# 0xPolygon/go-ibft

Hardware: AMD Instinct MI355X
Metric: committed_seal_verifies_per_sec (higher is better)
Workload: dtype u32

## Files before the change

### go-ibft_amd/build.py

```python
from __future__ import annotations

import os
import subprocess

HERE = os.path.dirname(os.path.abspath(__file__))
CSRC = os.path.join(HERE, "csrc")
LIB = os.path.join(CSRC, "libibftgpu.so")
SOURCES = ["ibftgpu.hip", "kernels.hip.h", "recover_dev.h", "verify_dev.h", "wave_fe_dev.h", "wire_dev.h", "cert_wave_dev.h", "modinv_dev.h",
           "sign_dev.h", "secp256k1_dev.h", "keccak_dev.h", os.path.join("..", "..", "include", "ibftgpu.h")]
CODEGEN_FLAGS = ["-mllvm", "-amdgpu-sched-strategy=max-ilp"]
EXTRA_FLAGS = ([] if os.environ.get("IBFT_NO_CODEGEN_FLAGS") == "1" else CODEGEN_FLAGS) + os.environ.get("IBFT_HIPCC_FLAGS", "").split()
HOST_HARNESS = os.path.join(CSRC, "libdev_arith_host.so")
WAVE_HARNESS = os.path.join(CSRC, "libdev_wave_host.so")
CERT_WAVE_HARNESS = os.path.join(CSRC, "libdev_cert_wave_host.so")


def _digest(deps: list[str], extra: str = "") -> str:
    import hashlib
    h = hashlib.sha256(extra.encode())
    for d in deps:
        with open(os.path.join(CSRC, d), "rb") as f:
            h.update(d.encode() + b"\0" + f.read() + b"\0")
    return h.hexdigest()


def _file_sha256(path: str) -> str:
    import hashlib
    h = hashlib.sha256()
    with open(path, "rb") as f:
        for blk in iter(lambda: f.read(1 << 20), b""):
            h.update(blk)
    return h.hexdigest()


def _read_stamp(target: str) -> list[str]:
    try:
        with open(target + ".stamp") as f:
            return f.read().split("\n")
    except OSError:
        return []


# ... 50 lines not shown


def build_lib(force: bool = False, verbose: bool = False) -> str:
    cmd = ["hipcc", "--offload-arch=gfx950", "-O3", "-std=c++17", *EXTRA_FLAGS, "-shared", "-fPIC",
           "-o", LIB, os.path.join(CSRC, "ibftgpu.hip"), "-ldl"]
    stamp_extra = " ".join(cmd[:-3]) + (" +phase_align" if PHASE_ALIGN else "")
    deps = SOURCES + ([os.path.join("..", "phase_align.py")] if PHASE_ALIGN else [])
    retry = PHASE_ALIGN and (build_info(LIB)["flavour"] or "").startswith("phase_align_failed")
    if force or retry or _stale(LIB, deps, stamp_extra):
        done = False
        flavour = "one_step"
        if PHASE_ALIGN:
            try:
                if verbose:
                    print(" ".join(cmd), "  (+ phase_align.py between device assembly and code object)", flush=True)
                _build_lib_phase_aligned(verbose)
                done = True
                flavour = "phase_align"
            except Exception as e:
                print(f"build: phase-aligned build failed ({e}); building with hipcc in one step", flush=True)
                flavour = "phase_align_failed: " + " ".join(str(e).split())[:300]
        if not done:
            if verbose:
                print(" ".join(cmd), flush=True)
            subprocess.check_call(cmd, cwd=CSRC)
        _mark(LIB, deps, stamp_extra, flavour)
    return LIB


DEVTEST = os.path.join(CSRC, "libibft_devtest.so")


def build_devtest(force: bool = False) -> str:
    deps = ["devtest.hip", "recover_dev.h", "modinv_dev.h", "secp256k1_dev.h", "keccak_dev.h", "wave_fe_dev.h", "verify_dev.h"]
    if force or _stale(DEVTEST, deps):
        subprocess.check_call(["hipcc", "--offload-arch=gfx950", "-O3", "-std=c++17", "-shared", "-fPIC", "-w",
                               "-o", DEVTEST, os.path.join(CSRC, "devtest.hip")], cwd=CSRC)
        _mark(DEVTEST, deps)
    return DEVTEST


def build_host_harness(force: bool = False) -> str:
    deps = ["host_arith_harness.hip", "sign_dev.h", "recover_dev.h", "modinv_dev.h", "secp256k1_dev.h", "keccak_dev.h", "wire_dev.h", "verify_dev.h"]
    if force or _stale(HOST_HARNESS, deps):
        subprocess.check_call(["hipcc", "--cuda-host-only", "-O2", "-std=c++17", "-shared", "-fPIC",
                               "-o", HOST_HARNESS, os.path.join(CSRC, "host_arith_harness.hip")], cwd=CSRC)
        _mark(HOST_HARNESS, deps)
    return HOST_HARNESS


def build_wave_harness(force: bool = False) -> str:
    deps = ["host_wave_harness.hip", "wave_fe_dev.h", "wave_emul.h", "recover_dev.h", "verify_dev.h",
            "modinv_dev.h", "secp256k1_dev.h", "keccak_dev.h"]
    if force or _stale(WAVE_HARNESS, deps):
        subprocess.check_call(["hipcc", "--cuda-host-only", "-O2", "-std=c++17", "-shared", "-fPIC",
                               "-o", WAVE_HARNESS, os.path.join(CSRC, "host_wave_harness.hip")], cwd=CSRC)
        _mark(WAVE_HARNESS, deps)
    return WAVE_HARNESS


def build_cert_wave_harness(force: bool = False) -> str:
    deps = ["host_cert_wave_harness.hip", "cert_wave_dev.h", "wave_emul.h", "wire_dev.h", "keccak_dev.h"]
    if force or _stale(CERT_WAVE_HARNESS, deps):
        subprocess.check_call(["hipcc", "--cuda-host-only", "-O2", "-std=c++17", "-shared", "-fPIC",
                               "-o", CERT_WAVE_HARNESS, os.path.join(CSRC, "host_cert_wave_harness.hip")], cwd=CSRC)
        _mark(CERT_WAVE_HARNESS, deps)
    return CERT_WAVE_HARNESS


PROPOSAL_DIGEST_HARNESS = os.path.join(CSRC, "libdev_proposal_digest_host.so")


def build_proposal_digest_harness(force: bool = False) -> str:
    deps = ["host_proposal_digest_harness.hip", "cert_wave_dev.h", "wave_emul.h", "wire_dev.h", "keccak_dev.h"]
    if force or _stale(PROPOSAL_DIGEST_HARNESS, deps):
        subprocess.check_call(["hipcc", "--cuda-host-only", "-O2", "-std=c++17", "-shared", "-fPIC",
                               "-o", PROPOSAL_DIGEST_HARNESS, os.path.join(CSRC, "host_proposal_digest_harness.hip")], cwd=CSRC)
        _mark(PROPOSAL_DIGEST_HARNESS, deps)
    return PROPOSAL_DIGEST_HARNESS


BLOCK_SETS_HARNESS = os.path.join(CSRC, "libdev_block_sets_host.so")


def build_block_sets_harness(force: bool = False) -> str:
    deps = ["host_block_sets_harness.hip", "recover_dev.h", "modinv_dev.h", "secp256k1_dev.h", "keccak_dev.h"]
    if force or _stale(BLOCK_SETS_HARNESS, deps):
        subprocess.check_call(["hipcc", "--cuda-host-only", "-O2", "-std=c++17", "-shared", "-fPIC",
                               "-o", BLOCK_SETS_HARNESS, os.path.join(CSRC, "host_block_sets_harness.hip")], cwd=CSRC)
        _mark(BLOCK_SETS_HARNESS, deps)
    return BLOCK_SETS_HARNESS


BLOCK_HEAD_HARNESS = os.path.join(CSRC, "libdev_block_head_host.so")


def build_block_head_harness(force: bool = False) -> str:
    deps = ["host_block_head_harness.hip", "recover_dev.h", "modinv_dev.h", "secp256k1_dev.h", "keccak_dev.h"]
    if force or _stale(BLOCK_HEAD_HARNESS, deps):
        subprocess.check_call(["hipcc", "--cuda-host-only", "-O2", "-std=c++17", "-shared", "-fPIC",
                               "-o", BLOCK_HEAD_HARNESS, os.path.join(CSRC, "host_block_head_harness.hip")], cwd=CSRC)
        _mark(BLOCK_HEAD_HARNESS, deps)
# ... 6 lines not shown
```

### go-ibft_amd/csrc/devtest.hip

```cpp
#include <hip/hip_runtime.h>
#include <stdint.h>

#include "modinv_dev.h"
#include "recover_dev.h"
#include "secp256k1_dev.h"

using namespace secp;

__global__ void devtest_kernel(int op, int n, const uint8_t *a, const uint8_t *b, uint8_t *out) {
  int i = blockIdx.x * blockDim.x + threadIdx.x;
  if (i >= n) return;
  u256 x = from_be32(a + 32 * i), y = from_be32(b + 32 * i);
  u256 r = zero256();
  switch (op) {
    case 0: r = fe_to_u256(fe_mul(fe_from_u256(x), fe_from_u256(y))); break;
    case 1: r = fe_to_u256(fe_sqr(fe_from_u256(x))); break;
    case 2: r = fe_to_u256(fe_inv(fe_from_u256(x))); break;
    case 3: r = fe_to_u256(fe_inv_safegcd(fe_from_u256(x))); break;
    case 4: r = sc_canon(sc_mul(sc_from_u256(x), sc_from_u256(y))); break;
    case 5: r = sc_canon(sc_inv(sc_from_u256(x))); break;
    case 6: r = sc_canon(sc_inv_safegcd(sc_from_u256(x))); break;
    case 7: r = fe_to_u256(fe_sqrt_candidate(fe_from_u256(x))); break;
    case 8: {
      glv_split s = sc_split_lambda(x);
// ... 131 lines not shown
}
__device__ __forceinline__ wv::wjac devtest_load_pt(const uint32_t *src, const wv::wk &k) {
  const uint32_t *r = src + 31 * k.row;
  wv::wjac p;
  p.x = k.li < 10 ? r[k.li] : 0u;
  p.y = k.li < 10 ? r[10 + k.li] : 0u;
  p.z = k.li < 10 ? r[20 + k.li] : 0u;
  p.inf = r[30] != 0;
  return p;
}
__global__ void __launch_bounds__(64) devtest_wave_pt_kernel(int op, const uint32_t *pp, const uint32_t *qq, uint32_t *out) {
  const wv::wk k = wv::wk_init();
  wv::wjac p = devtest_load_pt(pp + 124 * blockIdx.x, k), q = devtest_load_pt(qq + 124 * blockIdx.x, k), r;
  switch (op) {
    case 0: r = wv::wjac_dbl(p, k); break;
    case 1: r = wv::wjac_add(p, q, k); break;
    case 2: r = wv::wjac_add_aff(p, wv::waff{q.x, q.y}, k); break;
    default: r = wv::wjac_add(p, wv::wjac_lane_xor(p, 16), k); break;
  }
  uint32_t *o = out + 124 * blockIdx.x + 31 * k.row;
  if (k.li < 10) {
    o[k.li] = r.x;
    o[10 + k.li] = r.y;
    o[20 + k.li] = r.z;
  }
  if (k.li == 0) o[30] = r.inf ? 1u : 0u;
}
template <int STOP>
__global__ void __launch_bounds__(64) devtest_wave_recover_kernel(const uint32_t *gtab, const uint8_t *dig, const uint8_t *sig65,
                                                                uint32_t flags, uint8_t *out) {
  const int i = blockIdx.x;
  uint32_t addr[5] = {0, 0, 0, 0, 0};
  aff Q;
  bool ok = wv::recover_pubkey_wave<STOP>(gtab, from_be32(dig + 32 * i), from_be32(sig65 + 65 * i), from_be32(sig65 + 65 * i + 32),
                                    sig65[65 * i + 64], flags, addr, Q);
  uint8_t *o = out + (size_t)24 * (64 * i + threadIdx.x);
  for (int k = 0; k < 5; k++) reinterpret_cast<uint32_t *>(o)[k] = addr[k];
  o[20] = ok ? 1 : 0;
}

template <typename T>
static T *dev_copy(const T *h, size_t n) {
  T *d = nullptr;
  if (hipMalloc(&d, n * sizeof(T)) != hipSuccess) return nullptr;
  (void)hipMemcpy(d, h, n * sizeof(T), hipMemcpyHostToDevice);
  return d;
}
extern "C" int devtest_wave_fe(int op, int jobs, const uint32_t *a, const uint32_t *b, uint32_t *out) {
  uint32_t *da = dev_copy(a, (size_t)40 * jobs), *db = dev_copy(b, (size_t)40 * jobs), *dout;
  if (!da || !db || hipMalloc(&dout, (size_t)256 * jobs) != hipSuccess) return -1;
  devtest_wave_fe_kernel<<<jobs, 64>>>(op, da, db, dout);
  int rc = hipDeviceSynchronize() == hipSuccess ? 0 : -2;
  (void)hipMemcpy(out, dout, (size_t)256 * jobs, hipMemcpyDeviceToHost);
  (void)hipFree(da); (void)hipFree(db); (void)hipFree(dout);
  return rc;
}
extern "C" int devtest_wave_pt(int op, int jobs, const uint32_t *p, const uint32_t *q, uint32_t *out) {
  uint32_t *dp = dev_copy(p, (size_t)124 * jobs), *dq = dev_copy(q, (size_t)124 * jobs), *dout;
  if (!dp || !dq || hipMalloc(&dout, (size_t)496 * jobs) != hipSuccess) return -1;
  (void)hipMemset(dout, 0, (size_t)496 * jobs);
  devtest_wave_pt_kernel<<<jobs, 64>>>(op, dp, dq, dout);
  int rc = hipDeviceSynchronize() == hipSuccess ? 0 : -2;
  (void)hipMemcpy(out, dout, (size_t)496 * jobs, hipMemcpyDeviceToHost);
  (void)hipFree(dp); (void)hipFree(dq); (void)hipFree(dout);
  return rc;
}
extern "C" int devtest_wave_recover(int n, const uint8_t *dig, const uint8_t *sig65, uint32_t flags, uint8_t *out) {
  uint32_t *dg;
// ... 110 lines not shown
  if (!dd || !ds || hipMalloc(&dout, (size_t)24 * n) != hipSuccess) return -1;
  devtest_gtab_kernel<<<(ibftk::GTAB_WINDOWS * ibftk::GTAB_ENTRIES + 63) / 64, 64>>>(dg);
  hipEvent_t e0, e1;
  (void)hipEventCreate(&e0); (void)hipEventCreate(&e1);
  const int waves = (n + 3) / 4, blocks = (waves + 3) / 4;
  for (int reps = 1; reps <= max_reps; reps++)
    for (int t = 0; t < 3; t++) {
      (void)hipEventRecord(e0, 0);
      devtest_rows_repeat_kernel<<<blocks, 256>>>(dg, dd, ds, (uint32_t)n, reps, dout);
      (void)hipEventRecord(e1, 0);
      (void)hipEventSynchronize(e1);
      (void)hipEventElapsedTime(&ms[reps - 1], e0, e1);
    }
  int rc = hipDeviceSynchronize() == hipSuccess ? 0 : -2;
  (void)hipFree(dd); (void)hipFree(ds); (void)hipFree(dout); (void)hipFree(dg);
  return rc;
}

struct stamp_sync {
  uint64_t *st;
  uint32_t *cnt;
  __device__ void operator()() const {
    const uint64_t a = __builtin_amdgcn_s_memrealtime();
    __syncthreads();
    const uint64_t b = __builtin_amdgcn_s_memrealtime();
    if (__lane_id() == 0) {
      const uint32_t i = *cnt;
      st[1 + 2 * i] = a;
      st[2 + 2 * i] = b;
      *cnt = i + 1;
    }
  }
};
__global__ void __launch_bounds__(512) devtest_rows_pair_kernel(const uint32_t *gtab, const uint8_t *dig, const uint8_t *sig65,
                                                              uint32_t n, uint8_t *out, uint64_t *stamps) {
  __shared__ uint32_t row_tab[4][wv::ROW_TAB_SLOTS * 64];
  __shared__ wv::rows_pair_shared sh[4];
  __shared__ uint32_t cnt[8];
  const uint32_t w = threadIdx.x >> 6, lane = threadIdx.x & 63u, slot = w & 3u;
  uint64_t *st = stamps + (size_t)(blockIdx.x * 8 + w) * 8;
  if (lane == 0) {
    cnt[w] = 0;
    st[0] = __builtin_amdgcn_s_memrealtime();
  }
  const stamp_sync sync{st, &cnt[w]};
  const uint32_t row_raw = (blockIdx.x * 4 + slot) * 4u + (lane >> 4);
  const uint32_t i = row_raw < n ? row_raw : n - 1;
  const u256 r = from_be32(sig65 + 65 * i), s = from_be32(sig65 + 65 * i + 32);
  if (w >= 4) {
    wv::recover_helper_row(gtab, from_be32(dig + 32 * i), r, s, &sh[slot], sync);
    if (lane == 0) st[5] = __builtin_amdgcn_s_memrealtime();
    return;
  }
  uint32_t addr[5] = {0, 0, 0, 0, 0};
  aff Q;
  const bool ok = wv::recover_pubkey_row<99, true>(gtab, zero256(), r, s, sig65[65 * i + 64], 0, addr, Q, row_tab[slot], &sh[slot], sync);
  if (lane == 0) st[5] = __builtin_amdgcn_s_memrealtime();
  if ((lane & 15u) == 0 && row_raw < n) {
    uint8_t *o = out + (size_t)24 * i;
    for (int k = 0; k < 5; k++) reinterpret_cast<uint32_t *>(o)[k] = addr[k];
    o[20] = ok ? 1 : 0;
  }
}
extern "C" int devtest_rows_pair_stamps(int n, const uint8_t *dig, const uint8_t *sig65, uint8_t *out24, uint64_t *stamps8,
                                        float *ms) {
  if (n <= 0 || n % 16 != 0) return -3;
  uint32_t *dg;
  size_t gbytes = (size_t)ibftk::GTAB_WINDOWS * ibftk::GTAB_ENTRIES * ibftk::GTAB_ENTRY_DWORDS * 4;
  if (hipMalloc(&dg, gbytes) != hipSuccess) return -1;
  const int blocks = n / 16;
  const size_t st_words = (size_t)blocks * 8 * 8;
  uint8_t *dd = dev_copy(dig, (size_t)32 * n), *ds = dev_copy(sig65, (size_t)65 * n), *dout;
  uint64_t *dst;
  if (!dd || !ds || hipMalloc(&dout, (size_t)24 * n) != hipSuccess || hipMalloc(&dst, st_words * 8) != hipSuccess) return -1;
  devtest_gtab_kernel<<<(ibftk::GTAB_WINDOWS * ibftk::GTAB_ENTRIES + 63) / 64, 64>>>(dg);
  hipEvent_t e0, e1;
  (void)hipEventCreate(&e0); (void)hipEventCreate(&e1);
  for (int rep = 0; rep < 3; rep++) {
    (void)hipEventRecord(e0, 0);
    devtest_rows_pair_kernel<<<blocks, 512>>>(dg, dd, ds, (uint32_t)n, dout, dst);
    (void)hipEventRecord(e1, 0);
    (void)hipEventSynchronize(e1);
    (void)hipEventElapsedTime(ms, e0, e1);
  }
  int rc = hipDeviceSynchronize() == hipSuccess ? 0 : -2;
  if (rc == 0) {
    (void)hipMemcpy(out24, dout, (size_t)24 * n, hipMemcpyDeviceToHost);
    (void)hipMemcpy(stamps8, dst, st_words * 8, hipMemcpyDeviceToHost);
  }
  (void)hipFree(dd); (void)hipFree(ds); (void)hipFree(dout); (void)hipFree(dst); (void)hipFree(dg);
  return rc;
}
```

### go-ibft_amd/csrc/host_wave_harness.hip

```cpp
#define IBFT_GTAB_BITS 8
#define IBFT_WAVE_EMUL 1
#include <hip/hip_runtime.h>
#include <stdint.h>
#include <string.h>

#include <vector>

#include "wave_fe_dev.h"

using secp::u256;

static std::vector<uint32_t> g_gtab;

namespace {

struct mul_job {
  const uint32_t *a, *b;
  uint32_t *out;
  int op;
};
void lane_mul(void *p) {
  mul_job *j = (mul_job *)p;
  const wv::wk k = wv::wk_init();
  const uint32_t a = k.li < 10 ? j->a[k.row * 10 + k.li] : 0u;
// ... 16 lines not shown
struct pt_job {
  const uint32_t *p, *q;
  uint32_t *out;
  int op;
};
wv::wjac load_pt(const uint32_t *src, const wv::wk &k) {
  const uint32_t *r = src + 31 * k.row;
  wv::wjac p;
  p.x = k.li < 10 ? r[k.li] : 0u;
  p.y = k.li < 10 ? r[10 + k.li] : 0u;
  p.z = k.li < 10 ? r[20 + k.li] : 0u;
  p.inf = r[30] != 0;
  return p;
}
void lane_pt(void *vp) {
  pt_job *j = (pt_job *)vp;
  const wv::wk k = wv::wk_init();
  wv::wjac p = load_pt(j->p, k), q = load_pt(j->q, k), r;
  switch (j->op) {
    case 0: r = wv::wjac_dbl(p, k); break;
    case 1: r = wv::wjac_add(p, q, k); break;
    case 2: r = wv::wjac_add_aff(p, wv::waff{q.x, q.y}, k); break;
    default: r = wv::wjac_add(p, wv::wjac_lane_xor(p, 16), k); break;
  }
  uint32_t *o = j->out + 31 * k.row;
  if (k.li < 10) {
    o[k.li] = r.x;
    o[10 + k.li] = r.y;
    o[20 + k.li] = r.z;
  }
  if (k.li == 0) o[30] = r.inf ? 1u : 0u;
}

struct rec_job {
  const uint8_t *hash32, *sig65;
  uint32_t flags;
  uint8_t *addr20;
  int *ok;
};
void lane_rec(void *vp) {
  rec_job *j = (rec_job *)vp;
  u256 z = secp::from_be32(j->hash32), r = secp::from_be32(j->sig65), s = secp::from_be32(j->sig65 + 32);
  uint32_t a[5];
  secp::aff Q;
  bool ok = wv::recover_pubkey_wave(g_gtab.data(), z, r, s, j->sig65[64], j->flags, a, Q);
  const int l = wave_emul::lane();
  memcpy(j->addr20 + 20 * l, a, 20);
  j->ok[l] = ok ? 1 : 0;
}

struct rec2_job {
  const uint8_t *hash32, *sig65;
  uint32_t flags;
  uint8_t *addr20;
  int *ok;
  wv::pair_shared *sh;
};
void lane_rec2_helper(void *vp) {
  rec2_job *j = (rec2_job *)vp;
  u256 z = secp::from_be32(j->hash32), r = secp::from_be32(j->sig65), s = secp::from_be32(j->sig65 + 32);
  wv::recover_helper_wave(g_gtab.data(), z, r, s, j->sh, wv::no_sync());
}
void lane_rec2_main(void *vp) {
  rec2_job *j = (rec2_job *)vp;
  u256 z = secp::from_be32(j->hash32), r = secp::from_be32(j->sig65), s = secp::from_be32(j->sig65 + 32);
  uint32_t a[5];
  secp::aff Q;
  bool ok = wv::recover_pubkey_wave<99, true>(g_gtab.data(), z, r, s, j->sig65[64], j->flags, a, Q, j->sh, wv::no_sync());
  const int l = wave_emul::lane();
  memcpy(j->addr20 + 20 * l, a, 20);
  j->ok[l] = ok ? 1 : 0;
}

struct pre_job {
  const uint32_t *x;
  uint32_t *out;
  int ndbl;
};
void lane_prefix(void *vp) {
  pre_job *j = (pre_job *)vp;
  const wv::wk k = wv::wk_init();
  const uint32_t x = k.li < 10 ? j->x[k.li] : 0u;
  const uint32_t w = wv::wfe_weak(wv::wfe_mul(wv::wfe_sqr(x, k), x, k) + (k.li == 0 ? 7u : 0u), k);
  uint32_t PX = wv::wfe_mul(w, x, k), PY = wv::wfe_sqr(w, k), PZ, root;
  wv::prefix_and_sqrt(PX, PY, PZ, root, w, j->ndbl, k);
  const int l = wave_emul::lane();
  j->out[l] = PX;
  j->out[64 + l] = PY;
  j->out[128 + l] = PZ;
  j->out[192 + l] = root;
}

struct rec4_job {
  const uint8_t *hash32x4, *sig65x4;
  uint8_t *addr20;
  int *ok;
};
void lane_rec4(void *vp) {
  rec4_job *j = (rec4_job *)vp;
  const int l = wave_emul::lane(), row = l >> 4;
  const uint8_t *h = j->hash32x4 + 32 * row, *sg = j->sig65x4 + 65 * row;
// ... 167 lines not shown
```

### go-ibft_amd/csrc/kernels.hip.h

```cpp
#pragma once
#include <hip/hip_runtime.h>
#include <stdint.h>

#include "recover_dev.h"
#include "verify_dev.h"
#include "sign_dev.h"
#include "wave_fe_dev.h"
#include "wire_dev.h"
#include "cert_wave_dev.h"

namespace ibftk {

using secp::aff;
using secp::jac;
using secp::u256;

constexpr int ROWS_PER_BLOCK = 64;


constexpr int GATHER_MAX = 12;
constexpr int GATHER_BLOCK_BYTES = 256 * 16;
constexpr uint32_t GATHER_DIGEST_LDS = 32 * 1024;
struct gather_args {
  const uint8_t *src[GATHER_MAX];
// ... 735 lines not shown
  const uint32_t lane = threadIdx.x & 63u;
  if (row >= a.n) return;
  if (a.warm_done && a.warm_done[row] != 0) return;
  uint32_t want[5];
  int vi = -1;
  if (MODE != MODE_EMIT) {
#pragma unroll
    for (int i = 0; i < 5; i++) want[i] = reinterpret_cast<const uint32_t *>(a.signer20 + 20ull * row)[i];
    vi = valset_lookup(a.vtab, a.vslot_mask, want);
  }
  const bool pre = a.pre_flags && a.pre_flags[row] != 0;
  if (MODE == MODE_EMIT) {
    if (pre) {
      if (lane == 0) emit_store_none(a, row);
      return;
    }
  } else {
    if (lane == 0) a.vidx[row] = vi;
    if (pre || vi < 0) return;
  }
  const u256 r = secp::from_be32(a.sig65 + 65ull * row);
  const u256 s = secp::from_be32(a.sig65 + 65ull * row + 32);
  const uint32_t v = a.sig65[65ull * row + 64];
  u256 z;
  if (MODE != MODE_SENDERS) {
    z = secp::from_be32(a.hash32 + 32ull * row);
  } else {
    uint64_t d[4];
    hash_range_dwords(a.payload + a.off[row], a.off[row + 1] - a.off[row], d);
    keccak::digest_to_limbs(d, z.v);
  }
  uint32_t got[5];
  aff Qa;
  bool ok = wv::recover_pubkey_wave(a.gtab, z, r, s, v, a.flags, got, Qa);
  if (MODE == MODE_EMIT) {
    const emitted e = emit_row(ok, false, got, a.vtab, a.vslot_mask);
    if (lane == 0) emit_store(a, row, e);
    ok = e.bit;
    vi = e.vi;
  } else {
#pragma unroll
    for (int i = 0; i < 5; i++) ok = ok && (got[i] == want[i]);
  }
  if (lane == 0 && ok) {
    learn_key(a, vi, Qa);
    atomicOr(reinterpret_cast<unsigned long long *>(a.mask + (row >> 6)), 1ull << (row & 63));
  }
}

constexpr int PAIRS_PER_BLOCK = 2;
template <int MODE>
__global__ void __launch_bounds__(128 * PAIRS_PER_BLOCK) ecrecover_wave2_kernel(recover_args a) {
  __shared__ wv::pair_shared sh[PAIRS_PER_BLOCK];
  const uint32_t w = threadIdx.x >> 6, lane = threadIdx.x & 63u;
  const uint32_t slot = w % PAIRS_PER_BLOCK;
  const bool helper = w >= PAIRS_PER_BLOCK;
  const uint32_t row_raw = blockIdx.x * PAIRS_PER_BLOCK + slot;
  const bool live = row_raw < a.n;
  const uint32_t row = live ? row_raw : a.n - 1;
  const bool done = a.warm_done && a.warm_done[row] != 0;
  uint32_t want[5];
  int vi = -1;
  if (MODE != MODE_EMIT) {
#pragma unroll
    for (int i = 0; i < 5; i++) want[i] = reinterpret_cast<const uint32_t *>(a.signer20 + 20ull * row)[i];
    vi = valset_lookup(a.vtab, a.vslot_mask, want);
  }
  const bool pre = a.pre_flags && a.pre_flags[row] != 0;
  if (MODE != MODE_EMIT && !helper && lane == 0 && live && !done) a.vidx[row] = vi;
  const bool active = live && !done && !pre && (MODE == MODE_EMIT || vi >= 0);
  auto sync = [] { __syncthreads(); };
  if (!active) {
    if (MODE == MODE_EMIT && !helper && lane == 0 && live && !done) emit_store_none(a, row);
    sync();
    sync();
    return;
  }
  const u256 r = secp::from_be32(a.sig65 + 65ull * row);
  const u256 s = secp::from_be32(a.sig65 + 65ull * row + 32);
  const uint32_t v = a.sig65[65ull * row + 64];
  u256 z;
  if (MODE != MODE_SENDERS) {
    z = secp::from_be32(a.hash32 + 32ull * row);
  } else {
    uint64_t d[4];
    hash_range_dwords(a.payload + a.off[row], a.off[row + 1] - a.off[row], d);
    keccak::digest_to_limbs(d, z.v);
  }
  if (helper) {
    wv::recover_helper_wave(a.gtab, z, r, s, &sh[slot], sync);
    return;
  }
  uint32_t got[5];
  aff Qa;
  bool ok = wv::recover_pubkey_wave<99, true>(a.gtab, z, r, s, v, a.flags, got, Qa, &sh[slot], sync);
  if (MODE == MODE_EMIT) {
    const emitted e = emit_row(ok, false, got, a.vtab, a.vslot_mask);
    if (lane == 0) emit_store(a, row, e);
    ok = e.bit;
    vi = e.vi;
  } else {
#pragma unroll
    for (int i = 0; i < 5; i++) ok = ok && (got[i] == want[i]);
  }
  if (lane == 0 && ok) {
    learn_key(a, vi, Qa);
    atomicOr(reinterpret_cast<unsigned long long *>(a.mask + (row >> 6)), 1ull << (row & 63));
  }
}

template <int MODE>
__global__ void __launch_bounds__(64 * WAVE_KERNEL_WAVES) __attribute__((amdgpu_waves_per_eu(1, 2))) ecrecover_rows_kernel(recover_args a) {
  const uint32_t wave = blockIdx.x * WAVE_KERNEL_WAVES + (threadIdx.x >> 6);
  const uint32_t lane = threadIdx.x & 63u;
  if (wave * 4u >= a.n) return;
  const uint32_t row_raw = wave * 4u + (lane >> 4);
  const bool live = row_raw < a.n;
  const uint32_t row = live ? row_raw : a.n - 1;
  uint32_t want[5];
  int vi = -1;
  if (MODE != MODE_EMIT) {
#pragma unroll
    for (int i = 0; i < 5; i++) want[i] = reinterpret_cast<const uint32_t *>(a.signer20 + 20ull * row)[i];
    vi = valset_lookup(a.vtab, a.vslot_mask, want);
  }
  const bool pre = a.pre_flags && a.pre_flags[row] != 0;
  const bool done = a.warm_done && a.warm_done[row] != 0;
  const bool need = live && !done;
// ... 1253 lines not shown
```

### go-ibft_amd/csrc/wave_fe_dev.h

```cpp
#pragma once
#include "modinv_dev.h"
#include "recover_dev.h"
#include "verify_dev.h"
#if !defined(__HIP_DEVICE_COMPILE__) && defined(IBFT_WAVE_EMUL)
#include "wave_emul.h"
#endif

#if defined(__HIP_DEVICE_COMPILE__)
#define WVF __host__ __device__ __forceinline__
#else
#define WVF __host__ __device__ inline
#endif

namespace wv {

using secp::aff;
using secp::fe;
using secp::jac;
using secp::M26;
using secp::u256;

HD uint32_t lane_id() {
#if defined(__HIP_DEVICE_COMPILE__)
  return __lane_id();
// ... 674 lines not shown
  r.y = secp::fe_normalize(secp::fe_mul(p.y, secp::fe_mul(zi2, zi)));
  return !(p.inf || secp::fe_is_zero(p.z));
}

WVF waff gen_window_point(const uint32_t *__restrict__ gtab, const u256 &u1, int t, const wk &k) {
  constexpr int WPR = ibftk::GTAB_WINDOWS / 4;
  const int win = (int)k.row * WPR + t;
  const int bit = win * ibftk::GTAB_BITS;
  const uint32_t dgt = (u1.v[bit >> 5] >> (bit & 31)) & (uint32_t)(ibftk::GTAB_ENTRIES - 1);
  const uint32_t *e = gtab + (size_t)ibftk::GTAB_ENTRY_DWORDS * ((size_t)win * ibftk::GTAB_ENTRIES + dgt);
  const uint32_t ld = k.li < 10 ? k.li : 0u;
  waff pt;
  pt.x = e[ld] & k.act;
  pt.y = e[10 + ld] & k.act;
  return pt;
}
WVF wjac gen_windows_wave(const uint32_t *__restrict__ gtab, const u256 &u1, wjac acc, waff first, const wk &k) {
  constexpr int WPR = ibftk::GTAB_WINDOWS / 4;
  waff cur = first;
#pragma unroll 1
  for (int t = 0; t < WPR; t++) {
    const waff nxt = gen_window_point(gtab, u1, t + 1 < WPR ? t + 1 : t, k);
    const int bit = ((int)k.row * WPR + t) * ibftk::GTAB_BITS;
    const uint32_t dgt = (u1.v[bit >> 5] >> (bit & 31)) & (uint32_t)(ibftk::GTAB_ENTRIES - 1);
    const wjac sum = wjac_add_aff(acc, cur, k);
    acc = wjac_select(dgt != 0, sum, acc);
    cur = nxt;
  }
  return acc;
}
WVF wjac gen_windows_wave(const uint32_t *__restrict__ gtab, const u256 &u1, wjac acc, const wk &k) {
  return gen_windows_wave(gtab, u1, acc, gen_window_point(gtab, u1, 0, k), k);
}
struct pair_shared {
  uint32_t k1[4], k2[4];
  uint32_t neg;
  uint32_t ginf;
  uint32_t gx[16], gy[16], gz[16];
};
struct no_sync {
  HD void operator()() const {}
};
template <int STOP = 99, bool PAIR = false, class SYNC = no_sync>
WVF bool recover_pubkey_wave(const uint32_t *__restrict__ gtab, const u256 &z_raw, const u256 &r, const u256 &s,
                            uint32_t v, uint32_t flags, uint32_t addr[5], aff &Qa, const pair_shared *sh = nullptr,
                            SYNC sync = SYNC()) {
#define WV_STAGE(n, keep)     \
  if (STOP == (n)) {          \
    addr[0] = (keep);         \
    return ok;                \
  }
  const wk k = wk_init();
  bool ok = ibftk::sig_in_range(r, s, v, flags);
  const fe rx = secp::fe_from_u256(r);
  const uint32_t x = scatter(rx, k);
  const uint32_t one = k.li == 0 ? 1u : 0u;
  const uint32_t w = wfe_weak(wfe_mul(wfe_sqr(x, k), x, k) + (k.li == 0 ? 7u : 0u), k);
  const uint32_t X0 = wfe_mul(w, x, k), Y0 = wfe_sqr(w, k);
  uint32_t PX = X0, PY = Y0, PZ, yc;
  prefix_and_sqrt(PX, PY, PZ, yc, w, 64, k);
  WV_STAGE(1, PX ^ PY ^ PZ ^ yc)
  u256 u1 = secp::zero256();
  secp::glv_split sp;
  waff gfirst = waff{0u, 0u};
  if constexpr (PAIR) {
    sync();
    sp.k1 = sp.k2 = secp::zero256();
#pragma unroll
    for (int i = 0; i < 4; i++) {
      sp.k1.v[i] = sh->k1[i];
      sp.k2.v[i] = sh->k2[i];
    }
    sp.neg1 = (sh->neg & 1u) != 0;
    sp.neg2 = (sh->neg & 2u) != 0;
  } else {
    const secp::sc rinv = secp::sc_from_u256(modinv_wave<secp::ModN>(r, k));
    u1 = secp::sc_neg_canon(secp::sc_canon(secp::sc_mul(secp::sc_from_u256(z_raw), rinv)));
    const u256 u2 = secp::sc_canon(secp::sc_mul(secp::sc_from_u256(s), rinv));
    gfirst = gen_window_point(gtab, u1, 0, k);
// ... 58 lines not shown
    const uint32_t mag = (uint32_t)(dg < 0 ? -dg : dg);
    waff q = waff{AX[1], AY[1]};
#pragma unroll
    for (int e = 2; e <= 8; e++) {
      q.x = mag == (uint32_t)e ? AX[e] : q.x;
      q.y = mag == (uint32_t)e ? AY[e] : q.y;
    }
    q.y = dg < 0 ? wfe_neg1(q.y, k) : q.y;
    const wjac sum = wjac_add_aff<true>(acc, q, k);
    acc = wjac_select(mag != 0, sum, acc);
  }
  acc.z = wfe_mul(acc.z, Zc, k);
  WV_STAGE(4, acc.x ^ acc.y ^ acc.z ^ yc ^ u1.v[0])
  ok = ok && wfe_is_zero(wfe_sqr(yc, k) + wfe_neg1(w, k));
  fe y = secp::fe_normalize(gather(yc));
  y = secp::l26_select((y.n[0] & 1u) != v, secp::fe_normalize_weak(secp::fe_neg(y, 1)), y);
  acc.z = wfe_mul(acc.z, scatter(y, k), k);
  if constexpr (!PAIR) acc = gen_windows_wave(gtab, u1, acc, gfirst, k);
  acc = wjac_add(acc, wjac_lane_xor(acc, 16), k);
  acc = wjac_add(acc, wjac_lane_xor(acc, 32), k);
  if constexpr (PAIR) {
    sync();
    wjac g;
    g.x = sh->gx[k.li];
    g.y = sh->gy[k.li];
    g.z = sh->gz[k.li];
    g.inf = sh->ginf != 0;
    acc = wjac_add(acc, g, k);
  }
  WV_STAGE(5, acc.x ^ acc.y ^ acc.z)
  const jac Q = wjac_gather(acc);
  ok = jac_to_aff_wave(Qa, Q, k) && ok;
  WV_STAGE(6, Qa.x.n[0] ^ Qa.y.n[1])
  u256 qx = secp::l26_to_u256(Qa.x), qy = secp::l26_to_u256(Qa.y);
  keccak::address_from_xy(qx.v, qy.v, addr);
  return ok;
#undef WV_STAGE
}

template <class SYNC>
WVF void recover_helper_wave(const uint32_t *__restrict__ gtab, const u256 &z_raw, const u256 &r, const u256 &s, pair_shared *sh,
                             SYNC sync) {
  const wk k = wk_init();
  const secp::sc rinv = secp::sc_from_u256(modinv_wave<secp::ModN>(r, k));
  const u256 u1 = secp::sc_neg_canon(secp::sc_canon(secp::sc_mul(secp::sc_from_u256(z_raw), rinv)));
  const u256 u2 = secp::sc_canon(secp::sc_mul(secp::sc_from_u256(s), rinv));
  const secp::glv_split sp = secp::sc_split_lambda(u2);
  if (lane_id() == 0) {
#pragma unroll
    for (int i = 0; i < 4; i++) {
      sh->k1[i] = sp.k1.v[i];
      sh->k2[i] = sp.k2.v[i];
    }
    sh->neg = (sp.neg1 ? 1u : 0u) | (sp.neg2 ? 2u : 0u);
  }
  sync();
  wjac acc = gen_windows_wave(gtab, u1, wjac_inf(), k);
  acc = wjac_add(acc, wjac_lane_xor(acc, 16), k);
  acc = wjac_add(acc, wjac_lane_xor(acc, 32), k);
  if (lane_id() < 16) {
    sh->gx[k.li] = acc.x;
    sh->gy[k.li] = acc.y;
    sh->gz[k.li] = acc.z;
  }
  if (lane_id() == 0) sh->ginf = acc.inf ? 1u : 0u;
  sync();
}

// ... 206 lines not shown
  for (int jd = 31; jd >= 0; jd--) {
    const int n1 = (int)((w1[jd >> 3] >> (4 * (jd & 7))) & 15u), n2 = (int)((w2[jd >> 3] >> (4 * (jd & 7))) & 15u);
    const int d1 = jd == 32 ? (int)(w1[4] & 1u) : n1 - 8, d2 = jd == 32 ? (int)(w2[4] & 1u) : n2 - 8;
    const uint32_t m1 = (uint32_t)(d1 < 0 ? -d1 : d1), m2 = (uint32_t)(d2 < 0 ? -d2 : d2);
    const int e1 = 3 * (int)((m1 ? m1 : 1u) - 1u), e2 = 3 * (int)((m2 ? m2 : 1u) - 1u);
    waff q1 = waff{WT(e1), WT(e1 + 1)}, q2 = waff{WT(e2 + 2), WT(e2 + 1)};
    if (jd < 32) {
#pragma unroll 1
      for (int d = 0; d < 4; d++) acc = wjac_dbl<true>(acc, k);
    }
    q1.y = ((d1 < 0) != sp.neg1) ? wfe_neg1(q1.y, k) : q1.y;
    q2.y = ((d2 < 0) != sp.neg2) ? wfe_neg1(q2.y, k) : q2.y;
    const wjac s1 = wjac_add_aff<true>(acc, q1, k);
    acc = wjac_select(m1 != 0, s1, acc);
    const wjac s2 = wjac_add_aff<true>(acc, q2, k);
    acc = wjac_select(m2 != 0, s2, acc);
  }
#undef WT
  acc.z = wfe_mul(acc.z, Zc, k);
  WV_STAGE(4, acc.x ^ acc.y ^ acc.z ^ u1.v[0])
  wjac accg;
  if constexpr (PAIR) {
    sync();
    accg.x = sh->gx[lane_];
    accg.y = sh->gy[lane_];
    accg.z = sh->gz[lane_];
    accg.inf = sh->ginf[lane_] != 0;
  } else {
    accg = rows_fixed_base(gtab, u1, k);
  }
  WV_STAGE(5, acc.x ^ acc.y ^ acc.z ^ accg.x ^ accg.z)
  ok = rows_finish_deferred(Qa, accg, acc, rhs, v, k) && ok;
  WV_STAGE(6, Qa.x.n[0] ^ Qa.y.n[1])
  u256 qx = secp::l26_to_u256(Qa.x), qy = secp::l26_to_u256(Qa.y);
  keccak::address_from_xy(qx.v, qy.v, addr);
  return ok;
#undef WV_STAGE
}

template <class SYNC>
WVF void recover_helper_row(const uint32_t *__restrict__ gtab, const u256 &z_raw, const u256 &r, const u256 &s,
                            rows_pair_shared *sh, SYNC sync) {
  const wk k = wk_init();
  const secp::sc rinv = secp::sc_from_u256(modinv_wave<secp::ModN>(r, k));
  const u256 u1 = secp::sc_neg_canon(secp::sc_canon(secp::sc_mul(secp::sc_from_u256(z_raw), rinv)));
  const u256 u2 = secp::sc_canon(secp::sc_mul(secp::sc_from_u256(s), rinv));
  const secp::glv_split sp = secp::sc_split_lambda(u2);
  if (k.li == 0) {
    uint32_t *sr = sh->sc[k.row];
#pragma unroll
    for (int i = 0; i < 4; i++) {
      sr[i] = sp.k1.v[i];
      sr[4 + i] = sp.k2.v[i];
    }
    sr[8] = (sp.neg1 ? 1u : 0u) | (sp.neg2 ? 2u : 0u);
  }
  sync();
  const wjac accg = rows_fixed_base<true>(gtab, u1, k);
  const uint32_t l = lane_id();
  sh->gx[l] = accg.x;
  sh->gy[l] = accg.y;
  sh->gz[l] = accg.z;
  sh->ginf[l] = accg.inf ? 1u : 0u;
  sync();
}

WVF bool verify_known_wave(const uint32_t *__restrict__ gtab, const uint32_t *__restrict__ qtab_v, const u256 &z_raw,
                           const u256 &r, const u256 &s, uint32_t v, uint32_t flags) {
// ... 43 lines not shown
```

Before: 13.77 million.

## Compute Keccak address hash cooperatively across a 16-lane row using LDS

Replaces the per-lane scalar Keccak-f (every lane redundantly hashing the recovered pubkey) with a row-cooperative version. Each of 16 lanes holds one state column, theta reductions use row shuffles, and rho/pi permutation goes through an LDS scratch buffer with wave barriers. Scratch is added as new shared arrays in the wave kernels and reuses the window table in the row path. This reduces register pressure and per-lane ALU work in the final hashing stage, at the cost of extra LDS traffic, shared memory, and sync per round.

```diff
diff --git a/go-ibft_amd/build.py b/go-ibft_amd/build.py
--- a/go-ibft_amd/build.py
+++ b/go-ibft_amd/build.py
@@ -7,7 +7,7 @@
 CSRC = os.path.join(HERE, "csrc")
 LIB = os.path.join(CSRC, "libibftgpu.so")
 SOURCES = ["ibftgpu.hip", "kernels.hip.h", "recover_dev.h", "verify_dev.h", "wave_fe_dev.h", "wire_dev.h", "cert_wave_dev.h", "modinv_dev.h",
-           "sign_dev.h", "secp256k1_dev.h", "keccak_dev.h", os.path.join("..", "..", "include", "ibftgpu.h")]
+           "sign_dev.h", "secp256k1_dev.h", "keccak_dev.h", "keccak_row_dev.h", os.path.join("..", "..", "include", "ibftgpu.h")]
 CODEGEN_FLAGS = ["-mllvm", "-amdgpu-sched-strategy=max-ilp"]
 EXTRA_FLAGS = ([] if os.environ.get("IBFT_NO_CODEGEN_FLAGS") == "1" else CODEGEN_FLAGS) + os.environ.get("IBFT_HIPCC_FLAGS", "").split()
 HOST_HARNESS = os.path.join(CSRC, "libdev_arith_host.so")
@@ -124,7 +124,7 @@
 
 
 def build_devtest(force: bool = False) -> str:
-    deps = ["devtest.hip", "recover_dev.h", "modinv_dev.h", "secp256k1_dev.h", "keccak_dev.h", "wave_fe_dev.h", "verify_dev.h"]
+    deps = ["devtest.hip", "recover_dev.h", "modinv_dev.h", "secp256k1_dev.h", "keccak_dev.h", "keccak_row_dev.h", "wave_fe_dev.h", "verify_dev.h"]
     if force or _stale(DEVTEST, deps):
         subprocess.check_call(["hipcc", "--offload-arch=gfx950", "-O3", "-std=c++17", "-shared", "-fPIC", "-w",
                                "-o", DEVTEST, os.path.join(CSRC, "devtest.hip")], cwd=CSRC)
@@ -143,7 +143,7 @@
 
 def build_wave_harness(force: bool = False) -> str:
     deps = ["host_wave_harness.hip", "wave_fe_dev.h", "wave_emul.h", "recover_dev.h", "verify_dev.h",
-            "modinv_dev.h", "secp256k1_dev.h", "keccak_dev.h"]
+            "modinv_dev.h", "secp256k1_dev.h", "keccak_dev.h", "keccak_row_dev.h"]
     if force or _stale(WAVE_HARNESS, deps):
         subprocess.check_call(["hipcc", "--cuda-host-only", "-O2", "-std=c++17", "-shared", "-fPIC",
                                "-o", WAVE_HARNESS, os.path.join(CSRC, "host_wave_harness.hip")], cwd=CSRC)
@@ -160,6 +160,19 @@
     return CERT_WAVE_HARNESS
 
 
+ROW_KECCAK_HARNESS = os.path.join(CSRC, "libdev_row_keccak_host.so")
+
+
+def build_row_keccak_harness(force: bool = False) -> str:
+    deps = ["host_row_keccak_harness.hip", "keccak_row_dev.h", "wave_fe_dev.h", "wave_emul.h", "recover_dev.h", "verify_dev.h",
+            "modinv_dev.h", "secp256k1_dev.h", "keccak_dev.h"]
+    if force or _stale(ROW_KECCAK_HARNESS, deps):
+        subprocess.check_call(["hipcc", "--cuda-host-only", "-O2", "-std=c++17", "-shared", "-fPIC",
+                               "-o", ROW_KECCAK_HARNESS, os.path.join(CSRC, "host_row_keccak_harness.hip")], cwd=CSRC)
+        _mark(ROW_KECCAK_HARNESS, deps)
+    return ROW_KECCAK_HARNESS
+
+
 PROPOSAL_DIGEST_HARNESS = os.path.join(CSRC, "libdev_proposal_digest_host.so")
 
 
diff --git a/go-ibft_amd/csrc/devtest.hip b/go-ibft_amd/csrc/devtest.hip
--- a/go-ibft_amd/csrc/devtest.hip
+++ b/go-ibft_amd/csrc/devtest.hip
@@ -187,8 +187,9 @@
   const int i = blockIdx.x;
   uint32_t addr[5] = {0, 0, 0, 0, 0};
   aff Q;
+  __shared__ uint32_t kscr[wv::KROW_SCRATCH_DWORDS];
   bool ok = wv::recover_pubkey_wave<STOP>(gtab, from_be32(dig + 32 * i), from_be32(sig65 + 65 * i), from_be32(sig65 + 65 * i + 32),
-                                    sig65[65 * i + 64], flags, addr, Q);
+                                    sig65[65 * i + 64], flags, addr, Q, kscr);
   uint8_t *o = out + (size_t)24 * (64 * i + threadIdx.x);
   for (int k = 0; k < 5; k++) reinterpret_cast<uint32_t *>(o)[k] = addr[k];
   o[20] = ok ? 1 : 0;
@@ -365,6 +366,7 @@
     }
   }
 };
+template <int STOP>
 __global__ void __launch_bounds__(512) devtest_rows_pair_kernel(const uint32_t *gtab, const uint8_t *dig, const uint8_t *sig65,
                                                               uint32_t n, uint8_t *out, uint64_t *stamps) {
   __shared__ uint32_t row_tab[4][wv::ROW_TAB_SLOTS * 64];
@@ -387,7 +389,7 @@
   }
   uint32_t addr[5] = {0, 0, 0, 0, 0};
   aff Q;
-  const bool ok = wv::recover_pubkey_row<99, true>(gtab, zero256(), r, s, sig65[65 * i + 64], 0, addr, Q, row_tab[slot], &sh[slot], sync);
+  const bool ok = wv::recover_pubkey_row<STOP, true>(gtab, zero256(), r, s, sig65[65 * i + 64], 0, addr, Q, row_tab[slot], &sh[slot], sync);
   if (lane == 0) st[5] = __builtin_amdgcn_s_memrealtime();
   if ((lane & 15u) == 0 && row_raw < n) {
     uint8_t *o = out + (size_t)24 * i;
@@ -395,8 +397,8 @@
     o[20] = ok ? 1 : 0;
   }
 }
-extern "C" int devtest_rows_pair_stamps(int n, const uint8_t *dig, const uint8_t *sig65, uint8_t *out24, uint64_t *stamps8,
-                                        float *ms) {
+extern "C" int devtest_rows_pair_stamps_stop(int stop, int n, const uint8_t *dig, const uint8_t *sig65, uint8_t *out24,
+                                             uint64_t *stamps8, float *ms) {
   if (n <= 0 || n % 16 != 0) return -3;
   uint32_t *dg;
   size_t gbytes = (size_t)ibftk::GTAB_WINDOWS * ibftk::GTAB_ENTRIES * ibftk::GTAB_ENTRY_DWORDS * 4;
@@ -411,7 +413,10 @@
   (void)hipEventCreate(&e0); (void)hipEventCreate(&e1);
   for (int rep = 0; rep < 3; rep++) {
     (void)hipEventRecord(e0, 0);
-    devtest_rows_pair_kernel<<<blocks, 512>>>(dg, dd, ds, (uint32_t)n, dout, dst);
+    if (stop == 6)
+      devtest_rows_pair_kernel<6><<<blocks, 512>>>(dg, dd, ds, (uint32_t)n, dout, dst);
+    else
+      devtest_rows_pair_kernel<99><<<blocks, 512>>>(dg, dd, ds, (uint32_t)n, dout, dst);
     (void)hipEventRecord(e1, 0);
     (void)hipEventSynchronize(e1);
     (void)hipEventElapsedTime(ms, e0, e1);
@@ -424,3 +429,7 @@
   (void)hipFree(dd); (void)hipFree(ds); (void)hipFree(dout); (void)hipFree(dst); (void)hipFree(dg);
   return rc;
 }
+extern "C" int devtest_rows_pair_stamps(int n, const uint8_t *dig, const uint8_t *sig65, uint8_t *out24, uint64_t *stamps8,
+                                        float *ms) {
+  return devtest_rows_pair_stamps_stop(99, n, dig, sig65, out24, stamps8, ms);
+}
diff --git a/go-ibft_amd/csrc/host_row_keccak_harness.hip b/go-ibft_amd/csrc/host_row_keccak_harness.hip
--- /dev/null
+++ b/go-ibft_amd/csrc/host_row_keccak_harness.hip
@@ -0,0 +1,44 @@
+#define IBFT_GTAB_BITS 8
+#define IBFT_WAVE_EMUL 1
+#include <hip/hip_runtime.h>
+#include <stdint.h>
+#include <string.h>
+
+#include "wave_fe_dev.h"
+
+namespace {
+
+struct job {
+  const uint8_t *xy;
+  uint8_t *addr;
+  uint32_t *scr;
+};
+void lane_addr(void *vp) {
+  job *j = (job *)vp;
+  const uint32_t lane = wv::lane_id(), row = lane >> 4;
+  const secp::fe X = secp::fe_from_u256(secp::from_be32(j->xy + 64 * row));
+  const secp::fe Y = secp::fe_from_u256(secp::from_be32(j->xy + 64 * row + 32));
+  uint32_t a[5];
+  wv::address_from_xy_row(X, Y, a, j->scr);
+  memcpy(j->addr + 20 * lane, a, 20);
+}
+
+}
+
+extern "C" void row_keccak_addresses(const uint8_t *xy, int n_waves, uint8_t *addr) {
+  static uint32_t scr[wv::KROW_SCRATCH_DWORDS];
+  for (int w = 0; w < n_waves; w++) {
+    memset(scr, w & 1 ? 0xA5 : 0, sizeof scr);
+    job j{xy + 256 * w, addr + 1280 * w, scr};
+    wave_emul::run(lane_addr, &j);
+  }
+}
+
+extern "C" void lane_keccak_address(const uint8_t *xy, uint8_t *addr) {
+  const secp::u256 x = secp::from_be32(xy), y = secp::from_be32(xy + 32);
+  uint32_t a[5];
+  keccak::address_from_xy(x.v, y.v, a);
+  memcpy(addr, a, 20);
+}
+
+extern "C" int row_keccak_scratch_dwords() { return wv::KROW_SCRATCH_DWORDS; }
diff --git a/go-ibft_amd/csrc/host_wave_harness.hip b/go-ibft_amd/csrc/host_wave_harness.hip
--- a/go-ibft_amd/csrc/host_wave_harness.hip
+++ b/go-ibft_amd/csrc/host_wave_harness.hip
@@ -72,6 +72,7 @@
   if (k.li == 0) o[30] = r.inf ? 1u : 0u;
 }
 
+uint32_t g_kscr[wv::KROW_SCRATCH_DWORDS];
 struct rec_job {
   const uint8_t *hash32, *sig65;
   uint32_t flags;
@@ -83,7 +84,7 @@
   u256 z = secp::from_be32(j->hash32), r = secp::from_be32(j->sig65), s = secp::from_be32(j->sig65 + 32);
   uint32_t a[5];
   secp::aff Q;
-  bool ok = wv::recover_pubkey_wave(g_gtab.data(), z, r, s, j->sig65[64], j->flags, a, Q);
+  bool ok = wv::recover_pubkey_wave(g_gtab.data(), z, r, s, j->sig65[64], j->flags, a, Q, g_kscr);
   const int l = wave_emul::lane();
   memcpy(j->addr20 + 20 * l, a, 20);
   j->ok[l] = ok ? 1 : 0;
@@ -106,7 +107,7 @@
   u256 z = secp::from_be32(j->hash32), r = secp::from_be32(j->sig65), s = secp::from_be32(j->sig65 + 32);
   uint32_t a[5];
   secp::aff Q;
-  bool ok = wv::recover_pubkey_wave<99, true>(g_gtab.data(), z, r, s, j->sig65[64], j->flags, a, Q, j->sh, wv::no_sync());
+  bool ok = wv::recover_pubkey_wave<99, true>(g_gtab.data(), z, r, s, j->sig65[64], j->flags, a, Q, g_kscr, j->sh, wv::no_sync());
   const int l = wave_emul::lane();
   memcpy(j->addr20 + 20 * l, a, 20);
   j->ok[l] = ok ? 1 : 0;
diff --git a/go-ibft_amd/csrc/keccak_row_dev.h b/go-ibft_amd/csrc/keccak_row_dev.h
--- /dev/null
+++ b/go-ibft_amd/csrc/keccak_row_dev.h
@@ -0,0 +1,120 @@
+#pragma once
+#include "keccak_dev.h"
+
+namespace wv {
+
+constexpr int KROW_ROW_QWORDS = 56;
+constexpr int KROW_SCRATCH_DWORDS = 4 * KROW_ROW_QWORDS * 2;
+
+HD void wave_lds_sync() {
+#if defined(__HIP_DEVICE_COMPILE__)
+  __builtin_amdgcn_fence(__ATOMIC_ACQ_REL, "wavefront");
+  __builtin_amdgcn_wave_barrier();
+#elif defined(IBFT_WAVE_EMUL)
+  (void)wave_emul::xchg(0u, wave_emul::lane(), 0x700u);
+#endif
+}
+
+HD uint32_t krow_alignbit(uint32_t a, uint32_t b, uint32_t s) {
+#if defined(__HIP_DEVICE_COMPILE__)
+  return __builtin_amdgcn_alignbit(a, b, s);
+#else
+  return (uint32_t)((((uint64_t)a << 32) | b) >> (s & 31u));
+#endif
+}
+
+HD constexpr uint32_t krow_rot_pack(int a0, int a1, int a2, int a3, int a4) {
+  return (uint32_t)((64 - a0) & 63) | (uint32_t)((64 - a1) & 63) << 6 | (uint32_t)((64 - a2) & 63) << 12 |
+         (uint32_t)((64 - a3) & 63) << 18 | (uint32_t)((64 - a4) & 63) << 24;
+}
+
+WVF void address_from_xy_row(const fe &X, const fe &Y, uint32_t addr[5], uint32_t *scr) {
+  const u256 qx = secp::l26_to_u256(X), qy = secp::l26_to_u256(Y);
+  const uint32_t lane = lane_id(), li = lane & 15u, row = lane >> 4;
+  const bool l0 = li == 0, l1 = li == 1;
+  uint32_t lo[5], hi[5];
+#pragma unroll
+  for (int x = 0; x < 5; x++) {
+    const uint32_t a_lo = x < 4 ? qx.v[7 - 2 * x] : qy.v[7], a_hi = x < 4 ? qx.v[6 - 2 * x] : qy.v[6];
+    const uint32_t b_lo = x < 3 ? qy.v[5 - 2 * x] : 0u, b_hi = x < 3 ? qy.v[4 - 2 * x] : 0u;
+    lo[x] = keccak::bswap32(l0 ? a_lo : (l1 ? b_lo : 0u));
+    hi[x] = keccak::bswap32(l0 ? a_hi : (l1 ? b_hi : 0u));
+  }
+  lo[3] |= l1 ? 0x01u : 0u;
+  hi[1] |= li == 3 ? 0x80000000u : 0u;
+  const uint32_t R0 = krow_rot_pack(0, 1, 62, 28, 27), R1 = krow_rot_pack(36, 44, 6, 55, 20),
+                 R2 = krow_rot_pack(3, 10, 43, 25, 39), R3 = krow_rot_pack(41, 45, 15, 21, 8),
+                 R4 = krow_rot_pack(18, 2, 61, 56, 14);
+  const uint32_t rot = l0 ? R0 : (l1 ? R1 : (li == 2 ? R2 : (li == 3 ? R3 : R4)));
+  uint32_t rs[5];
+  bool swp[5];
+#pragma unroll
+  for (int x = 0; x < 5; x++) {
+    rs[x] = rot >> (6 * x);
+    swp[x] = (rot >> (6 * x + 5) & 1u) != 0;
+  }
+  const uint32_t m0 = l0 ? 0xFFFFFFFFu : 0u;
+  const bool plane = li < 5;
+  const uint32_t rbase = row * (uint32_t)KROW_ROW_QWORDS;
+  const uint32_t wr = rbase + li + (plane ? 0u : 20u);
+  const uint32_t y3 = (0x24130u >> (4u * (li & 7u))) & 7u;
+  uint32_t rd[5];
+#pragma unroll
+  for (int x = 0; x < 5; x++) {
+    const uint32_t t = (uint32_t)x + y3, src = t >= 5u ? t - 5u : t;
+    rd[x] = plane ? rbase + 5u * src + (uint32_t)x : wr + 5u * (uint32_t)x;
+  }
+#pragma unroll 1
+  for (int round = 0; round < 24; round++) {
+    uint32_t cl[5], ch[5];
+#pragma unroll
+    for (int x = 0; x < 5; x++) {
+      uint32_t a = lo[x], b = hi[x];
+      a ^= row_shr<1>(a);
+      b ^= row_shr<1>(b);
+      a ^= row_shr<2>(a);
+      b ^= row_shr<2>(b);
+      a ^= row_shr<4>(a);
+      b ^= row_shr<4>(b);
+      cl[x] = a;
+      ch[x] = b;
+    }
+#pragma unroll
+    for (int x = 0; x < 5; x++) {
+      const int p = (x + 4) % 5, n = (x + 1) % 5;
+      const uint32_t dl = cl[p] ^ krow_alignbit(cl[n], ch[n], 31u);
+      const uint32_t dh = ch[p] ^ krow_alignbit(ch[n], cl[n], 31u);
+      lo[x] ^= row_bcast<4>(dl);
+      hi[x] ^= row_bcast<4>(dh);
+    }
+#pragma unroll
+    for (int x = 0; x < 5; x++) {
+      const uint32_t a = swp[x] ? hi[x] : lo[x], b = swp[x] ? lo[x] : hi[x];
+      scr[2u * (wr + 5u * (uint32_t)x)] = krow_alignbit(b, a, rs[x]);
+      scr[2u * (wr + 5u * (uint32_t)x) + 1u] = krow_alignbit(a, b, rs[x]);
+    }
+    wave_lds_sync();
+    uint32_t bl[5], bh[5];
+#pragma unroll
+    for (int x = 0; x < 5; x++) {
+      bl[x] = scr[2u * rd[x]];
+      bh[x] = scr[2u * rd[x] + 1u];
+    }
+    wave_lds_sync();
+#pragma unroll
+    for (int x = 0; x < 5; x++) {
+      lo[x] = bl[x] ^ (~bl[(x + 1) % 5] & bl[(x + 2) % 5]);
+      hi[x] = bh[x] ^ (~bh[(x + 1) % 5] & bh[(x + 2) % 5]);
+    }
+    const uint64_t rc = keccak::rc(round);
+    lo[0] ^= (uint32_t)rc & m0;
+    hi[0] ^= (uint32_t)(rc >> 32) & m0;
+  }
+  addr[0] = row_bcast<0>(hi[1]);
+  addr[1] = row_bcast<0>(lo[2]);
+  addr[2] = row_bcast<0>(hi[2]);
+  addr[3] = row_bcast<0>(lo[3]);
+  addr[4] = row_bcast<0>(hi[3]);
+}
+
+}
diff --git a/go-ibft_amd/csrc/kernels.hip.h b/go-ibft_amd/csrc/kernels.hip.h
--- a/go-ibft_amd/csrc/kernels.hip.h
+++ b/go-ibft_amd/csrc/kernels.hip.h
@@ -791,7 +791,8 @@
   }
   uint32_t got[5];
   aff Qa;
-  bool ok = wv::recover_pubkey_wave(a.gtab, z, r, s, v, a.flags, got, Qa);
+  __shared__ uint32_t krow_scr[WAVE_KERNEL_WAVES][wv::KROW_SCRATCH_DWORDS];
+  bool ok = wv::recover_pubkey_wave(a.gtab, z, r, s, v, a.flags, got, Qa, krow_scr[threadIdx.x >> 6]);
   if (MODE == MODE_EMIT) {
     const emitted e = emit_row(ok, false, got, a.vtab, a.vslot_mask);
     if (lane == 0) emit_store(a, row, e);
@@ -811,6 +812,7 @@
 template <int MODE>
 __global__ void __launch_bounds__(128 * PAIRS_PER_BLOCK) ecrecover_wave2_kernel(recover_args a) {
   __shared__ wv::pair_shared sh[PAIRS_PER_BLOCK];
+  __shared__ uint32_t krow_scr[PAIRS_PER_BLOCK][wv::KROW_SCRATCH_DWORDS];
   const uint32_t w = threadIdx.x >> 6, lane = threadIdx.x & 63u;
   const uint32_t slot = w % PAIRS_PER_BLOCK;
   const bool helper = w >= PAIRS_PER_BLOCK;
@@ -852,7 +854,7 @@
   }
   uint32_t got[5];
   aff Qa;
-  bool ok = wv::recover_pubkey_wave<99, true>(a.gtab, z, r, s, v, a.flags, got, Qa, &sh[slot], sync);
+  bool ok = wv::recover_pubkey_wave<99, true>(a.gtab, z, r, s, v, a.flags, got, Qa, krow_scr[slot], &sh[slot], sync);
   if (MODE == MODE_EMIT) {
     const emitted e = emit_row(ok, false, got, a.vtab, a.vslot_mask);
     if (lane == 0) emit_store(a, row, e);
diff --git a/go-ibft_amd/csrc/wave_fe_dev.h b/go-ibft_amd/csrc/wave_fe_dev.h
--- a/go-ibft_amd/csrc/wave_fe_dev.h
+++ b/go-ibft_amd/csrc/wave_fe_dev.h
@@ -730,6 +730,10 @@
 WVF wjac gen_windows_wave(const uint32_t *__restrict__ gtab, const u256 &u1, wjac acc, const wk &k) {
   return gen_windows_wave(gtab, u1, acc, gen_window_point(gtab, u1, 0, k), k);
 }
+}
+#include "keccak_row_dev.h"
+namespace wv {
+
 struct pair_shared {
   uint32_t k1[4], k2[4];
   uint32_t neg;
@@ -741,8 +745,8 @@
 };
 template <int STOP = 99, bool PAIR = false, class SYNC = no_sync>
 WVF bool recover_pubkey_wave(const uint32_t *__restrict__ gtab, const u256 &z_raw, const u256 &r, const u256 &s,
-                            uint32_t v, uint32_t flags, uint32_t addr[5], aff &Qa, const pair_shared *sh = nullptr,
-                            SYNC sync = SYNC()) {
+                            uint32_t v, uint32_t flags, uint32_t addr[5], aff &Qa, uint32_t *kscr,
+                            const pair_shared *sh = nullptr, SYNC sync = SYNC()) {
 #define WV_STAGE(n, keep)     \
   if (STOP == (n)) {          \
     addr[0] = (keep);         \
@@ -867,8 +871,7 @@
   const jac Q = wjac_gather(acc);
   ok = jac_to_aff_wave(Qa, Q, k) && ok;
   WV_STAGE(6, Qa.x.n[0] ^ Qa.y.n[1])
-  u256 qx = secp::l26_to_u256(Qa.x), qy = secp::l26_to_u256(Qa.y);
-  keccak::address_from_xy(qx.v, qy.v, addr);
+  address_from_xy_row(Qa.x, Qa.y, addr, kscr);
   return ok;
 #undef WV_STAGE
 }
@@ -1141,8 +1144,8 @@
   WV_STAGE(5, acc.x ^ acc.y ^ acc.z ^ accg.x ^ accg.z)
   ok = rows_finish_deferred(Qa, accg, acc, rhs, v, k) && ok;
   WV_STAGE(6, Qa.x.n[0] ^ Qa.y.n[1])
-  u256 qx = secp::l26_to_u256(Qa.x), qy = secp::l26_to_u256(Qa.y);
-  keccak::address_from_xy(qx.v, qy.v, addr);
+  static_assert(KROW_SCRATCH_DWORDS <= ROW_TAB_SLOTS * 64, "the row Keccak's scratch lives in the window table");
+  address_from_xy_row(Qa.x, Qa.y, addr, wtab);
   return ok;
 #undef WV_STAGE
 }
```

Measured after the change: 13.93 million (median of 6 runs). 1.1% higher.
